# AntoineBlanot/LC2IS

Hardware: AMD Instinct MI355X
Metric: training-step images/sec (512x512, ADE20K-150) (higher is better)
Workload: dtype bf16; 1 GPU; BaseModelWithText ViT-B/16 + CLIP-text + decoder + fused head/CE train step, 512x512, 151 classes, text len 16, sgd; batch_per_gpu=32, global_batch=32, parallelism=dp1

## Files before the change

### include/lc2is_hip.h

```cpp
#ifndef LC2IS_HIP_H
#define LC2IS_HIP_H
#include <stddef.h>
#include <stdint.h>

#ifdef __cplusplus
extern "C" {
#endif

#define LC2IS_ACT_NONE 0
#define LC2IS_ACT_QUICK_GELU 1
#define LC2IS_ACT_RELU 2
#define LC2IS_ACT_DQUICK_GELU 3
#define LC2IS_ACT_DRELU 4
#define LC2IS_ACT_QUICK_GELU_GRAD 5
#define LC2IS_ACT_MUL_AUX 6
#define LC2IS_ACT_GELU_ERF 7
#define LC2IS_ACT_DGELU_ERF 8
#define LC2IS_ACT_ADD_AUX 9

#define LC2IS_INTERP_BICUBIC 0
#define LC2IS_INTERP_BILINEAR 1

typedef void* lc2is_stream_t;

// ... 108 lines not shown
  int C;
  int accumulate;
} lc2is_ln_partials;
int lc2is_layernorm_bwd_partials(int M, int C);
int lc2is_ln_partials_reduce(const lc2is_ln_partials* items, int n, lc2is_stream_t stream);

int lc2is_attention_fwd(const void* Q, int ldq, const void* K, int ldk, const void* V, int ldv, void* O,
                        int ldo, float* lse2, const float* kbias, int B, int H, int Sq, int Sk, int D,
                        float scale, int causal, lc2is_stream_t stream);

int lc2is_attention_bwd(const void* Q, int ldq, const void* K, int ldk, const void* V, int ldv,
                        const void* O, int ldo, const void* dO, int lddo, void* dQ, int lddq, void* dK,
                        int lddk, void* dV, int lddv, const float* lse2, float* delta, const float* kbias,
                        int B, int H, int Sq, int Sk, int D, float scale, int causal, lc2is_stream_t stream);

int lc2is_attention_fwd_dropout(const void* Q, int ldq, const void* K, int ldk, const void* V, int ldv, void* O,
                                int ldo, float* lse2, const float* kbias, int B, int H, int Sq, int Sk, int D,
                                float scale, int causal, float p_drop, unsigned long long seed, lc2is_stream_t stream);
int lc2is_attention_bwd_dropout(const void* Q, int ldq, const void* K, int ldk, const void* V, int ldv,
                                const void* O, int ldo, const void* dO, int lddo, void* dQ, int lddq, void* dK,
                                int lddk, void* dV, int lddv, const float* lse2, float* delta, const float* kbias,
                                int B, int H, int Sq, int Sk, int D, float scale, int causal, float p_drop,
                                unsigned long long seed, lc2is_stream_t stream);

int lc2is_dropout_rows_f32(const float* x, int ldx, const float* resid, int ldr, float* y32, int ldy, void* y16,
                           int ldy16, int M, int C, int rows_per_sample, float p, unsigned long long seed,
                           lc2is_stream_t stream);
int lc2is_dropout_rows_bf16(const void* x, int ldx, void* y, int ldy, int M, int C, float p, unsigned long long seed,
                            lc2is_stream_t stream);
int lc2is_dropout_mask(unsigned char* out, long rows, int cols, float p, unsigned long long seed, lc2is_stream_t stream);


int lc2is_shadow_refresh(const lc2is_shadow_desc* descs, int ndesc, int total_tiles, lc2is_stream_t stream);
int lc2is_cast_f32_bf16(const float* src, int ld_src, void* dst_bf16, int ld_dst, int M, int C,
                        lc2is_stream_t stream);
int lc2is_transpose_bf16(const void* src, int ld_src, void* dst, int ld_dst, int R, int C,
                         lc2is_stream_t stream);
int lc2is_transpose_bf16_batched(const void* src, int ld_src, long stride_src, void* dst, int ld_dst, long stride_dst,
                                 int R, int C, int batch, lc2is_stream_t stream);

int lc2is_patchify(const float* pixels, void* out_bf16, int ld_out, int B, int H, int W, int patch,
                   lc2is_stream_t stream);
int lc2is_vit_embed_fwd(const float* patch, int ld_patch, const float* cls, const float* pos, float* x,
                        int ldx, int B, int P, int C, lc2is_stream_t stream);
int lc2is_vit_embed_bwd(const float* dx, int ldx, float* dpos, float* dcls, void* dpatch_bf16, int ld_dpatch,
                        int B, int P, int C, int accumulate, lc2is_stream_t stream);
// ... 340 lines not shown
```

### lc2is_amd/nn/decoder.py

```python
from __future__ import annotations

import copy

import torch
from torch import nn

from .. import ops
from .base import (DropSites, HipModule, WgradBatch, drop_branch_add, drop_branch_grad16, grad_buf, linear_bwd_params,
                   require_cuda, vec_grad)


class _SelfAttnParams(nn.Module):
    def __init__(self, c, bias):
        super().__init__()
        self.in_proj_weight = nn.Parameter(torch.empty(3 * c, c))
        self.in_proj_bias = nn.Parameter(torch.zeros(3 * c)) if bias else None
        self.out_proj = nn.Linear(c, c, bias=bias)
        nn.init.xavier_uniform_(self.in_proj_weight)


class _CrossAttnParams(nn.Module):
    def __init__(self, c, ckv):
        super().__init__()
        self.q_proj_weight = nn.Parameter(torch.empty(c, c))
        self.k_proj_weight = nn.Parameter(torch.empty(c, ckv))
        self.v_proj_weight = nn.Parameter(torch.empty(c, ckv))
        self.in_proj_bias = nn.Parameter(torch.zeros(3 * c))
        self.out_proj = nn.Linear(c, c, bias=True)
        for w in (self.q_proj_weight, self.k_proj_weight, self.v_proj_weight):
            nn.init.xavier_uniform_(w)
        nn.init.zeros_(self.out_proj.bias)

# ... 46 lines not shown
    sa, ca = layer.self_attn, layer.multihead_attn
    s = dict(w_in=torch.empty(3 * C, C, **bf), w_inT=torch.empty(C, 3 * C, **bf),
             w_so=torch.empty(C, C, **bf), w_soT=torch.empty(C, C, **bf),
             w_q=torch.empty(C, C, **bf), w_qT=torch.empty(C, C, **bf),
             w_kv=torch.empty(2 * C, Ckv, **bf), w_kvT=torch.empty(Ckv, 2 * C, **bf),
             w_co=torch.empty(C, C, **bf), w_coT=torch.empty(C, C, **bf),
             w1=torch.empty(F, C, **bf), w1T=torch.empty(C, F, **bf),
             w2=torch.empty(C, F, **bf), w2T=torch.empty(F, C, **bf))
    e = [(sa.in_proj_weight, s["w_in"], s["w_inT"]), (sa.out_proj.weight, s["w_so"], s["w_soT"]),
         (ca.q_proj_weight, s["w_q"], s["w_qT"]),
         (ca.k_proj_weight, s["w_kv"][:C], s["w_kvT"][:, :C]), (ca.v_proj_weight, s["w_kv"][C:], s["w_kvT"][:, C:]),
         (ca.out_proj.weight, s["w_co"], s["w_coT"]),
         (layer.linear1.weight, s["w1"], s["w1T"]), (layer.linear2.weight, s["w2"], s["w2T"])]
    return s, e


def _layer_fwd(x, mem16, layer: DecoderLayer, s, B, Sq, Sk, kbias, save, ds: DropSites | None = None):
    C, H = layer.d_model, layer.nhead
    D = C // H
    scale = D ** -0.5
    sa, ca = layer.self_attn, layer.multihead_attn
    bq, bkv = ca.in_proj_bias[:C], ca.in_proj_bias[C:]
    nf = layer.norm_first
    sv = {}

    def ln(i, t, want_f32):
        n = getattr(layer, f"norm{i}")
        yb, yf, m, r = ops.layernorm_fwd(t, n.weight, n.bias, layer.eps, save_stats=save, out_bf16=True,
                                         out_f32=True if want_f32 else None)
        sv[f"ln{i}"] = (t, m, r)
        return yb, yf

    if nf:
        h1, _ = ln(1, x, False)
    else:
        h1 = ops.cast_bf16(x)
    qkv, _, _ = ops.gemm_nt(h1, s["w_in"], sa.in_proj_bias)
    pd = ds.p if ds is not None else 0.0
    o1, lse1 = ops.attention_fwd(qkv[:, :C], qkv[:, C:2 * C], qkv[:, 2 * C:], B, H, Sq, Sq, D, scale, save_lse=save,
                                 dropout_p=pd, seed=ds.seed("sa_p") if ds else 0)
    if ds is None:
        _, x1, _ = ops.gemm_nt(o1, s["w_so"], sa.out_proj.bias, resid=x, out_bf16=None, out_f32=True)
    else:
        _, br, _ = ops.gemm_nt(o1, s["w_so"], sa.out_proj.bias, out_bf16=None, out_f32=True)
        x1 = drop_branch_add(ds, "d1", br, x)
    if not nf:
        h2, x1 = ln(1, x1, True)
    if nf:
        h2, _ = ln(2, x1, False)
    q, _, _ = ops.gemm_nt(h2, s["w_q"], bq)
    kv, _, _ = ops.gemm_nt(mem16, s["w_kv"], bkv)
    o2, lse2 = ops.attention_fwd(q, kv[:, :C], kv[:, C:], B, H, Sq, Sk, D, scale, kbias=kbias, save_lse=save,
                                 dropout_p=pd, seed=ds.seed("ca_p") if ds else 0)
    if ds is None:
        _, x2, _ = ops.gemm_nt(o2, s["w_co"], ca.out_proj.bias, resid=x1, out_bf16=None, out_f32=True)
    else:
        _, br, _ = ops.gemm_nt(o2, s["w_co"], ca.out_proj.bias, out_bf16=None, out_f32=True)
        x2 = drop_branch_add(ds, "d2", br, x1)
    if not nf:
        h3, x2 = ln(2, x2, True)
    if nf:
        h3, _ = ln(3, x2, False)
    a, _, _ = ops.gemm_nt(h3, s["w1"], layer.linear1.bias, act=ops.ACT_RELU)
    if ds is None:
        _, x3, _ = ops.gemm_nt(a, s["w2"], layer.linear2.bias, resid=x2, out_bf16=None, out_f32=True)
    else:
        ops.dropout_rows_bf16(a, ds.p, ds.seed("ff"))
        _, br, _ = ops.gemm_nt(a, s["w2"], layer.linear2.bias, out_bf16=None, out_f32=True)
        x3 = drop_branch_add(ds, "d3", br, x2)
    if not nf:
        _, x3 = ln(3, x3, True)
    if save:
        sv.update(h1=h1, qkv=qkv, o1=o1, lse1=lse1, h2=h2, q=q, kv=kv, o2=o2, lse2=lse2, h3=h3, a=a, ds=ds)
    return x3, (sv if save else None)


def _layer_bwd(g32, g16, dmem32, mem16, layer, s, sv, B, Sq, Sk, kbias):
    with WgradBatch():
        return _layer_bwd_impl(g32, g16, dmem32, mem16, layer, s, sv, B, Sq, Sk, kbias)


def _layer_bwd_impl(g32, g16, dmem32, mem16, layer: DecoderLayer, s, sv, B, Sq, Sk, kbias):
    C, H = layer.d_model, layer.nhead
    D = C // H
    scale = D ** -0.5
    sa, ca = layer.self_attn, layer.multihead_attn
    nf = layer.norm_first

    def ln_bwd(i, dy, dres):
        n = getattr(layer, f"norm{i}")
        t, m, r = sv[f"ln{i}"]
        dg, accg = vec_grad(n.weight)
        db, _ = vec_grad(n.bias)
        a32, a16, _, _ = ops.layernorm_bwd(dy, t, n.weight, m, r, dres=dres, dgamma=dg, dbeta=db, accumulate=accg,
                                           need_param_grads=dg is not None)
        return a32, a16

    ds = sv.get("ds")
    pd = ds.p if ds is not None else 0.0
    if not nf:
        g32, g16 = ln_bwd(3, g32, None)
    gb16 = drop_branch_grad16(ds, "d3", g32, g16)
    linear_bwd_params(gb16, sv["a"], layer.linear2.weight, layer.linear2.bias)
    dz, _, _ = ops.gemm_nt(gb16, s["w2T"], None, act=ops.ACT_DRELU, aux_in=sv["a"])
    if ds is not None:
        ops.dropout_rows_bf16(dz, ds.p, ds.seeds["ff"])
    linear_bwd_params(dz, sv["h3"], layer.linear1.weight, layer.linear1.bias)
    if nf:
        dh3, _, _ = ops.gemm_nt(dz, s["w1T"], None)
        g32, g16 = ln_bwd(3, dh3, g32)
    else:
        _, g32, _ = ops.gemm_nt(dz, s["w1T"], None, resid=g32, out_bf16=None, out_f32=True)
        g32, g16 = ln_bwd(2, g32, None)
    gb16 = drop_branch_grad16(ds, "d2", g32, g16)
    linear_bwd_params(gb16, sv["o2"], ca.out_proj.weight, ca.out_proj.bias)
    do2, _, _ = ops.gemm_nt(gb16, s["w_coT"], None)
    q, kv = sv["q"], sv["kv"]
    dq = torch.empty_like(q)
    dkv = torch.empty_like(kv)
    ops.attention_bwd(q, kv[:, :C], kv[:, C:], sv["o2"], do2, sv["lse2"], B, H, Sq, Sk, D, scale, kbias=kbias, dq=dq,
                      dk=dkv[:, :C], dv=dkv[:, C:], dropout_p=pd, seed=ds.seeds["ca_p"] if ds else 0)
    gb, accb = vec_grad(ca.in_proj_bias)
    if ca.q_proj_weight.requires_grad:
        gw, acc = grad_buf(ca.q_proj_weight)
        ops.gemm_tn(dq, sv["h2"], gw, accumulate=acc)
        gw, acc = grad_buf(ca.k_proj_weight)
        ops.gemm_tn(dkv[:, :C], mem16, gw, accumulate=acc)
        gw, acc = grad_buf(ca.v_proj_weight)
        ops.gemm_tn(dkv[:, C:], mem16, gw, accumulate=acc)
    if gb is not None:
        ops.colsum(dq, gb[:C], accumulate=accb)
        ops.colsum(dkv, gb[C:], accumulate=accb)
    ops.gemm_nt(dkv, s["w_kvT"], None, resid=dmem32, out_bf16=None, out_f32=dmem32)
    if nf:
        dh2, _, _ = ops.gemm_nt(dq, s["w_qT"], None)
        g32, g16 = ln_bwd(2, dh2, g32)
    else:
        _, g32, _ = ops.gemm_nt(dq, s["w_qT"], None, resid=g32, out_bf16=None, out_f32=True)
        g32, g16 = ln_bwd(1, g32, None)
    gb16 = drop_branch_grad16(ds, "d1", g32, g16)
    linear_bwd_params(gb16, sv["o1"], sa.out_proj.weight, sa.out_proj.bias)
    do1, _, _ = ops.gemm_nt(gb16, s["w_soT"], None)
    qkv = sv["qkv"]
    dqkv = torch.empty_like(qkv)
    ops.attention_bwd(qkv[:, :C], qkv[:, C:2 * C], qkv[:, 2 * C:], sv["o1"], do1, sv["lse1"], B, H, Sq, Sq, D, scale,
                      dq=dqkv[:, :C], dk=dqkv[:, C:2 * C], dv=dqkv[:, 2 * C:], dropout_p=pd,
                      seed=ds.seeds["sa_p"] if ds else 0)
    linear_bwd_params(dqkv, sv["h1"], sa.in_proj_weight, sa.in_proj_bias)
    if nf:
        dh1, _, _ = ops.gemm_nt(dqkv, s["w_inT"], None)
        g32, g16 = ln_bwd(1, dh1, g32)
    else:
        _, g32, _ = ops.gemm_nt(dqkv, s["w_inT"], None, resid=g32, out_bf16=None, out_f32=True)
        g16 = ops.cast_bf16(g32)
# ... 101 lines not shown
```

### lc2is_amd/ops.py

```python
from __future__ import annotations

import ctypes as C
import math
import os

import torch

from . import _lib

ACT_NONE, ACT_QUICK_GELU, ACT_RELU, ACT_DQUICK_GELU, ACT_DRELU, ACT_QUICK_GELU_GRAD, ACT_MUL_AUX = 0, 1, 2, 3, 4, 5, 6
ACT_GELU_ERF, ACT_DGELU_ERF, ACT_ADD_AUX = 7, 8, 9

_P, _I, _F, _Z, _L, _U64 = C.c_void_p, C.c_int, C.c_float, C.c_size_t, C.c_long, C.c_ulonglong
_ARGTYPES = {
    "lc2is_gemm_nt_bf16": [_P, _I, _P, _I, _P, _P, _I, _P, _I, _P, _I, _P, _I, _P, _I, _I, _I, _I, _I, _I, _P],
    "lc2is_gemm_nt_plan": [_P, _I, _P, _I, _P, _P, _I, _P, _I, _P, _I, _P, _I, _P, _I, _I, _I, _I, _I, _I, _P, _I],
    "lc2is_gemm_nt_ln_xchg_bytes": [_I, _I],
    "lc2is_gemm_nt_ln_bf16": [_P, _I, _P, _I, _P, _P, _I, _P, _I, _P, _P, _F, _P, _I, _P, _P, _P, _Z, _I, _I, _I, _P],
    "lc2is_gemm_nt_bf16_batched": [_P, _I, _L, _P, _I, _L, _P, _I, _L, _P, _I, _L, _I, _I, _I, _I, _P],
    "lc2is_transpose_bf16_batched": [_P, _I, _L, _P, _I, _L, _I, _I, _I, _P],
    "lc2is_gemm_tn_workspace_bytes": [_I, _I, _I],
    "lc2is_gemm_tn_bf16": [_P, _I, _P, _I, _P, _I, _P, _I, _I, _I, _I, _P, _Z, _P],
    "lc2is_gemm_tn_plan": [_I, _I, _I, _P],
    "lc2is_gemm_tn_grouped_plan": [_P, _I, _P, _P, _I],
    "lc2is_colsum_workspace_bytes": [_I, _I],
    "lc2is_colsum_bf16": [_P, _I, _P, _I, _I, _I, _P, _Z, _P],
    "lc2is_layernorm_fwd": [_P, _I, _I, _P, _P, _P, _I, _P, _I, _P, _P, _I, _I, _F, _P],
    "lc2is_layernorm_bwd_partials": [_I, _I],
    "lc2is_ln_partials_reduce": [_P, _I, _P],
    "lc2is_layernorm_bwd_workspace_bytes": [_I, _I],
    "lc2is_layernorm_bwd": [_P, _I, _P, _I, _P, _I, _I, _P, _P, _P, _P, _I, _I, _P, _I, _P, _I, _P, _P, _I, _I, _I,
                            _P, _Z, _P],
    "lc2is_attention_fwd": [_P, _I, _P, _I, _P, _I, _P, _I, _P, _P, _I, _I, _I, _I, _I, _F, _I, _P],
    "lc2is_attention_bwd": [_P, _I, _P, _I, _P, _I, _P, _I, _P, _I, _P, _I, _P, _I, _P, _I, _P, _P, _P,
                            _I, _I, _I, _I, _I, _F, _I, _P],
    "lc2is_attention_fwd_dropout": [_P, _I, _P, _I, _P, _I, _P, _I, _P, _P, _I, _I, _I, _I, _I, _F, _I, _F, _U64, _P],
    "lc2is_attention_bwd_dropout": [_P, _I, _P, _I, _P, _I, _P, _I, _P, _I, _P, _I, _P, _I, _P, _I, _P, _P, _P,
                                    _I, _I, _I, _I, _I, _F, _I, _F, _U64, _P],
    "lc2is_dropout_rows_f32": [_P, _I, _P, _I, _P, _I, _P, _I, _I, _I, _I, _F, _U64, _P],
    "lc2is_dropout_rows_bf16": [_P, _I, _P, _I, _I, _I, _F, _U64, _P],
    "lc2is_dropout_mask": [_P, _L, _I, _F, _U64, _P],
    "lc2is_shadow_refresh": [_P, _I, _I, _P],
    "lc2is_set_cu_budget": [_I],
    "lc2is_get_cu_budget": [],
    "lc2is_cast_f32_bf16": [_P, _I, _P, _I, _I, _I, _P],
    "lc2is_transpose_bf16": [_P, _I, _P, _I, _I, _I, _P],
    "lc2is_patchify": [_P, _P, _I, _I, _I, _I, _I, _P],
    "lc2is_vit_embed_fwd": [_P, _I, _P, _P, _P, _I, _I, _I, _I, _P],
    "lc2is_vit_embed_bwd": [_P, _I, _P, _P, _P, _I, _I, _I, _I, _I, _P],
    "lc2is_text_embed_fwd": [_P, _P, _P, _P, _I, _I, _I, _I, _I, _P],
    "lc2is_text_embed_bwd": [_P, _P, _I, _P, _P, _I, _I, _I, _I, _I, _P],
    "lc2is_rows_copy_bf16": [_P, _I, _I, _P, _P, _I, _I, _I, _I, _I, _P],
    "lc2is_rows_copy_f32": [_P, _I, _I, _P, _P, _I, _I, _I, _I, _I, _P],
    "lc2is_sgd_step": [_P, _P, _P, _Z, _F, _F, _F, _F, _P],
    "lc2is_adamw_step": [_P, _P, _P, _P, _Z, _F, _F, _F, _F, _F, _I, _F, _P],
    "lc2is_grad_sumsq_blocks": [_Z],
    "lc2is_grad_sumsq_workspace_bytes": [_Z],
    "lc2is_grad_sumsq": [_P, _Z, _P, _Z, _P],
    "lc2is_optim_ctrl_update": [_P, _P, _P, _I, _P, _I, _F, _F, _I, _F, _F, _P],
    "lc2is_accum_add": [_P, _P, _P],
    "lc2is_optim_ctrl_update_accum": [_P, _P, _I, _P, _P, _I, _P, _I, _F, _F, _I, _F, _F, _P],
# ... 521 lines not shown
    while items:
        chunk, rest, seen = [], [], set()
        for it in items:
            outs = {t.data_ptr() for t in (it[3], it[4]) if t is not None}
            if len(chunk) < LN_PARTIALS_MAX and not (outs & seen) and not rest:
                chunk.append(it); seen |= outs
            else:
                rest.append(it)
        arr = (LnPartials * len(chunk))()
        for i, (ws, nparts, Cc, dg, db, acc) in enumerate(chunk):
            _chk(dg, torch.float32, "dgamma", 1); _chk(db, torch.float32, "dbeta", 1)
            arr[i] = LnPartials(_ptr(ws), _ptr(dg), _ptr(db), nparts, Cc, int(acc))
        rc = _fn("lc2is_ln_partials_reduce")(arr, len(chunk), _stream())
        _lib.check(rc, f"ln_partials_reduce n={len(chunk)}")
        items = rest


def ln_defer_end(prev):
    global _ln_defer
    ln_defer_flush()
    _ln_defer = prev


def attention_fwd(q: torch.Tensor, k: torch.Tensor, v: torch.Tensor, B: int, H: int, Sq: int, Sk: int, D: int,
                  scale: float, *, causal: bool = False, kbias: torch.Tensor | None = None,
                  save_lse: bool = True, out: torch.Tensor | None = None, dropout_p: float = 0.0, seed: int = 0):
    who, bf = "attention_fwd", torch.bfloat16
    dev, qs, ks = q.device, (B * Sq, H * D), (B * Sk, H * D)
    if _dims(who, q, "q", 2, bf) != qs:
        raise RuntimeError(f"lc2is_amd.attention_fwd: q must have shape {qs}, got {tuple(q.shape)}")
    _chk_op(who, k, "k", bf, ks, dev); _chk_op(who, v, "v", bf, ks, dev)
    _chk_op(who, kbias, "kbias", torch.float32, (B, Sk), dev, 4)
    o = out
    if o is None:
        o = torch.empty(qs, dtype=bf, device=dev)
    else:
        _chk_op(who, o, "out", bf, qs, dev); _chk_ld8(who, o, "out")
    lse = torch.empty((B, H, Sq), dtype=torch.float32, device=q.device) if save_lse else None
    if dropout_p > 0.0:
        rc = _fn("lc2is_attention_fwd_dropout")(_ptr(q), _ld(q), _ptr(k), _ld(k), _ptr(v), _ld(v), _ptr(o), _ld(o),
                                                _ptr(lse), _ptr(kbias), B, H, Sq, Sk, D, float(scale), int(causal),
                                                float(dropout_p), int(seed), _stream())
    else:
        rc = _fn("lc2is_attention_fwd")(_ptr(q), _ld(q), _ptr(k), _ld(k), _ptr(v), _ld(v), _ptr(o), _ld(o),
                                        _ptr(lse), _ptr(kbias), B, H, Sq, Sk, D, float(scale), int(causal),
                                        _stream())
    _lib.check(rc, f"attention_fwd B={B} H={H} Sq={Sq} Sk={Sk} D={D}")
    return o, lse


def attention_bwd(q, k, v, o, do, lse2, B: int, H: int, Sq: int, Sk: int, D: int, scale: float, *,
                  causal: bool = False, kbias: torch.Tensor | None = None, dq=None, dk=None, dv=None,
                  dropout_p: float = 0.0, seed: int = 0):
    who, bf = "attention_bwd", torch.bfloat16
    dev, qs, ks = q.device, (B * Sq, H * D), (B * Sk, H * D)
    if _dims(who, q, "q", 2, bf) != qs:
        raise RuntimeError(f"lc2is_amd.attention_bwd: q must have shape {qs}, got {tuple(q.shape)}")
    for t, n, s in ((k, "k", ks), (v, "v", ks), (o, "o", qs), (do, "do", qs)):
        if t is None:
            raise RuntimeError(f"lc2is_amd.attention_bwd: {n} is required")
        _chk_op(who, t, n, bf, s, dev)
    _chk_op(who, dq, "dq", bf, qs, dev); _chk_op(who, dk, "dk", bf, ks, dev); _chk_op(who, dv, "dv", bf, ks, dev)
    if dq is None:
        dq = torch.empty(qs, dtype=bf, device=dev)
    else:
        _chk_ld8(who, dq, "dq")
    dk = dk if dk is not None else torch.empty(ks, dtype=bf, device=dev)
    dv = dv if dv is not None else torch.empty(ks, dtype=bf, device=dev)
    if lse2 is None:
        raise RuntimeError("lc2is_amd.attention_bwd: lse2 is required")
    _chk_op(who, lse2, "lse2", torch.float32, (B, H, Sq), dev, 4); _chk_op(who, kbias, "kbias", torch.float32, (B, Sk), dev, 4)
    delta = torch.empty((B, H, Sq), dtype=torch.float32, device=dev)
    args = (_ptr(q), _ld(q), _ptr(k), _ld(k), _ptr(v), _ld(v), _ptr(o), _ld(o), _ptr(do), _ld(do), _ptr(dq), _ld(dq),
            _ptr(dk), _ld(dk), _ptr(dv), _ld(dv), _ptr(lse2), _ptr(delta), _ptr(kbias), B, H, Sq, Sk, D, float(scale),
            int(causal))
    if dropout_p > 0.0:
        rc = _fn("lc2is_attention_bwd_dropout")(*args, float(dropout_p), int(seed), _stream())
    else:
        rc = _fn("lc2is_attention_bwd")(*args, _stream())
    _lib.check(rc, f"attention_bwd B={B} H={H} Sq={Sq} Sk={Sk} D={D}")
    return dq, dk, dv


def dropout_rows_f32(x: torch.Tensor, p: float, seed: int, *, resid: torch.Tensor | None = None,
                     out_f32: torch.Tensor | bool | None = True, out_bf16: torch.Tensor | bool | None = None,
                     rows_per_sample: int = 0):
    who, dev = "dropout_rows_f32", x.device
    M, Cc = _dims(who, x, "x", 2, torch.float32)
    _chk_op(who, resid, "resid", torch.float32, (M, Cc), dev)
    yf = _out(out_f32, (M, Cc), torch.float32, dev)
    yb = _out(out_bf16, (M, Cc), torch.bfloat16, dev)
    if out_f32 is not True:
        _chk_op(who, yf, "out_f32", torch.float32, (M, Cc), dev)
    if out_bf16 is not True:
# ... 1630 lines not shown
```

Baseline: 1100 images/s.

## Add few-keys attention kernels and fuse decoder out-proj with layernorm

Adds specialised forward and backward attention kernels for short key sequences (Sk up to 64, D 64 or 96). Each block stages all of K and V for a head in LDS, computes the softmax in one pass with no online rescaling, and in backward accumulates dK/dV across query tiles in registers before a block reduction. This targets the decoder cross-attention over text tokens, where the generic flash kernel spends effort on key tiling. The decoder also fuses the out-projection GEMM with the residual add and the next layernorm, and moves the q-projection weight gradient into the batched wgrad group. Both new paths are behind env flags that default on.

```diff
diff --git a/include/lc2is_hip.h b/include/lc2is_hip.h
--- a/include/lc2is_hip.h
+++ b/include/lc2is_hip.h
@@ -154,6 +154,14 @@
                                 int lddk, void* dV, int lddv, const float* lse2, float* delta, const float* kbias,
                                 int B, int H, int Sq, int Sk, int D, float scale, int causal, float p_drop,
                                 unsigned long long seed, lc2is_stream_t stream);
+
+int lc2is_attention_fewkeys_fwd(const void* Q, int ldq, const void* K, int ldk, const void* V, int ldv, void* O,
+                                int ldo, float* lse2, const float* kbias, int B, int H, int Sq, int Sk, int D,
+                                float scale, int causal, lc2is_stream_t stream);
+int lc2is_attention_fewkeys_bwd(const void* Q, int ldq, const void* K, int ldk, const void* V, int ldv,
+                                const void* O, int ldo, const void* dO, int lddo, void* dQ, int lddq, void* dK,
+                                int lddk, void* dV, int lddv, const float* lse2, const float* kbias, int B, int H,
+                                int Sq, int Sk, int D, float scale, int causal, lc2is_stream_t stream);
 
 int lc2is_dropout_rows_f32(const float* x, int ldx, const float* resid, int ldr, float* y32, int ldy, void* y16,
                            int ldy16, int M, int C, int rows_per_sample, float p, unsigned long long seed,
diff --git a/lc2is_amd/csrc/attention_fewkeys.hip b/lc2is_amd/csrc/attention_fewkeys.hip
--- /dev/null
+++ b/lc2is_amd/csrc/attention_fewkeys.hip
@@ -0,0 +1,482 @@
+#include "attn_common.h"
+#include "lc2is_hip.h"
+
+namespace {
+
+constexpr float FK_LOG2E = 1.44269504088896341f;
+constexpr int FK_QB = 256;
+
+template <int D, int NKG> struct FkCfg {
+  static constexpr int PITCH = 2 * D + 16;
+  static constexpr int KR = 32 * NKG;
+  static constexpr int PP = 2 * KR + 16;
+  static constexpr int NKS = D / 16, NDT = D / 32, CPR = D / 8;
+  static constexpr int KV_BYTES = 2 * KR * PITCH + KR * 4;
+  static constexpr int FWD_LDS = KV_BYTES + 4 * 32 * PITCH;
+  static constexpr int BWD_WAVE = 64 * PITCH + 64 * PP;
+  static constexpr int RP = D + 4;
+  static constexpr int BWD_LDS = KV_BYTES + 4 * BWD_WAVE;
+  static_assert(2 * KR * RP * 4 <= BWD_LDS, "the dK / dV sum reuses the images");
+};
+
+__device__ __forceinline__ bf16x8_t fk_pack8(const f32x16_t& v, int r0) {
+  bf16x8_t o;
+#pragma unroll
+  for (int j = 0; j < 8; ++j) o[j] = (__bf16)v[r0 + j];
+  return o;
+}
+
+__device__ __forceinline__ float fk_dot8(const i32x4_t a, const i32x4_t b) {
+  float s = 0.f;
+#pragma unroll
+  for (int i = 0; i < 4; ++i) {
+    const unsigned x = (unsigned)a[i], y = (unsigned)b[i];
+    s += __builtin_bit_cast(float, x << 16) * __builtin_bit_cast(float, y << 16);
+    s += __builtin_bit_cast(float, x & 0xffff0000u) * __builtin_bit_cast(float, y & 0xffff0000u);
+  }
+  return s;
+}
+
+template <int D, int NKG>
+__device__ __forceinline__ void fk_stage_kv(char* smem, const bf16_t* K, int ldk, const bf16_t* V, int ldv, const float* kbias,
+                                            int B, int Sk, int b, int head, int tid) {
+  using C = FkCfg<D, NKG>;
+  const __amdgpu_buffer_rsrc_t rsK = make_rsrc(K, (unsigned)B * Sk * ldk * 2u);
+  const __amdgpu_buffer_rsrc_t rsV = make_rsrc(V, (unsigned)B * Sk * ldv * 2u);
+  for (int i = tid; i < C::KR * C::CPR; i += 256) {
+    const int r = i / C::CPR, ch = i - r * C::CPR;
+    const int ko = r < Sk ? ((b * Sk + r) * ldk + head * D + ch * 8) * 2 : -1;
+    const int vo = r < Sk ? ((b * Sk + r) * ldv + head * D + ch * 8) * 2 : -1;
+    *(i32x4_t*)(smem + r * C::PITCH + ch * 16) = __builtin_amdgcn_raw_buffer_load_b128(rsK, ko, 0, 0);
+    *(i32x4_t*)(smem + (C::KR + r) * C::PITCH + ch * 16) = __builtin_amdgcn_raw_buffer_load_b128(rsV, vo, 0, 0);
+  }
+  if (tid < C::KR) {
+    float* bias_l = (float*)(smem + 2 * C::KR * C::PITCH);
+    bias_l[tid] = tid < Sk ? (kbias ? kbias[(size_t)b * Sk + tid] * FK_LOG2E : 0.f) : -__builtin_inff();
+  }
+}
+
+template <int D, int PITCH>
+__device__ __forceinline__ void fk_store_rows(const char* img, bf16_t* dst, unsigned bytes, int tok0, int q0, int Sq, int ld,
+                                              int col0, int lane) {
+  constexpr int CPR = D / 8, RPI = 64 / CPR;
+  const __amdgpu_buffer_rsrc_t rs = make_rsrc(dst, bytes);
+  const int r_in = lane / CPR, ch = lane % CPR;
+  if (lane < RPI * CPR) {
+#pragma unroll
+    for (int it = 0; it < (32 + RPI - 1) / RPI; ++it) {
+      const int row = it * RPI + r_in;
+      if (row < 32) {
+        const i32x4_t v = *(const i32x4_t*)(img + row * PITCH + ch * 16);
+        const int off = (q0 + row < Sq) ? ((tok0 + q0 + row) * ld + col0 + ch * 8) * 2 : -1;
+        __builtin_amdgcn_raw_buffer_store_b128(v, rs, off, 0, 0);
+      }
+    }
+  }
+}
+
+struct FkFwdArgs {
+  const bf16_t* Q; int ldq;
+  const bf16_t* K; int ldk;
+  const bf16_t* V; int ldv;
+  bf16_t* O; int ldo;
+  float* lse2;
+  const float* kbias;
+  int B, H, Sq, Sk;
+  float scale_log2;
+};
+
+template <int D, int NKG>
+__global__ __launch_bounds__(256) void attn_fewkeys_fwd_kernel(FkFwdArgs p) {
+  using C = FkCfg<D, NKG>;
+  constexpr int PITCH = C::PITCH, KR = C::KR, NKS = C::NKS, NDT = C::NDT;
+  extern __shared__ __attribute__((aligned(16))) char smem[];
+  const int tid = threadIdx.x, lane = tid & 63;
+  const int wid = __builtin_amdgcn_readfirstlane(tid >> 6);
+  const int hh = lane >> 5, l31 = lane & 31;
+  const int q4 = (lane >> 2) & 3, p4 = lane & 3, cg = (lane >> 4) & 1;
+  const int nqb = (p.Sq + FK_QB - 1) / FK_QB;
+  const int bx = blockIdx.x % nqb, head = (blockIdx.x / nqb) % p.H, b = blockIdx.x / (nqb * p.H);
+  const float NEG_INF = -__builtin_inff();
+
+  fk_stage_kv<D, NKG>(smem, p.K, p.ldk, p.V, p.ldv, p.kbias, p.B, p.Sk, b, head, tid);
+  __syncthreads();
+
+  const unsigned smem_a = (unsigned)(size_t)LDS_PTR(smem);
+  const unsigned k_row = smem_a + l31 * PITCH + hh * 16;
+  const unsigned v_tr = smem_a + (KR + 4 * hh + q4) * PITCH + (16 * cg + 4 * p4) * 2;
+  char* obuf = smem + C::KV_BYTES + wid * (32 * PITCH);
+  float bias2[NKG][16];
+  {
+    const float* bias_l = (const float*)(smem + 2 * KR * PITCH);
+#pragma unroll
+    for (int g = 0; g < NKG; ++g)
+#pragma unroll
+      for (int c = 0; c < 4; ++c) {
+        const f32x4_t t = *(const f32x4_t*)(bias_l + 32 * g + 8 * c + 4 * hh);
+#pragma unroll
+        for (int j = 0; j < 4; ++j) bias2[g][4 * c + j] = t[j];
+      }
+  }
+
+  const __amdgpu_buffer_rsrc_t rsQ = make_rsrc(p.Q, (unsigned)p.B * p.Sq * p.ldq * 2u);
+  const int qend = (bx + 1) * FK_QB < p.Sq ? (bx + 1) * FK_QB : p.Sq;
+  auto load_q = [&](int q0, bf16x8_t (&qf)[NKS]) __attribute__((always_inline)) {
+    const int qr = q0 + l31;
+    const int off = (q0 < qend && qr < p.Sq) ? ((b * p.Sq + qr) * p.ldq + head * D + 8 * hh) * 2 : -1;
+#pragma unroll
+    for (int s = 0; s < NKS; ++s)
+      qf[s] = __builtin_bit_cast(bf16x8_t, __builtin_amdgcn_raw_buffer_load_b128(rsQ, off < 0 ? -1 : off + s * 32, 0, 0));
+  };
+
+  bf16x8_t qf[NKS], qn[NKS];
+  load_q(bx * FK_QB + wid * 32, qf);
+  for (int q0 = bx * FK_QB + wid * 32; q0 < qend; q0 += 128) {
+    load_q(q0 + 128, qn);
+    const int qrow = q0 + l31;
+    f32x16_t st[NKG];
+#pragma unroll
+    for (int g = 0; g < NKG; ++g) {
+#pragma unroll
+      for (int r = 0; r < 16; ++r) st[g][r] = 0.f;
+#pragma unroll
+      for (int s = 0; s < NKS; ++s)
+        st[g] = __builtin_amdgcn_mfma_f32_32x32x16_bf16(lds_read_b128(k_row + (unsigned)(32 * g * PITCH + 32 * s)), qf[s], st[g], 0, 0, 0);
+    }
+    float mx = NEG_INF;
+#pragma unroll
+    for (int g = 0; g < NKG; ++g)
+#pragma unroll
+      for (int r = 0; r < 16; ++r) {
+        st[g][r] = __builtin_fmaf(st[g][r], p.scale_log2, bias2[g][r]);
+        mx = fmaxf(mx, st[g][r]);
+      }
+    mx = fmaxf(mx, __shfl_xor(mx, 32, 64));
+    const float mref = mx == NEG_INF ? 0.f : mx;
+    float lsum = 0.f;
+#pragma unroll
+    for (int g = 0; g < NKG; ++g)
+#pragma unroll
+      for (int r = 0; r < 16; ++r) {
+        st[g][r] = __builtin_amdgcn_exp2f(st[g][r] - mref);
+        lsum += st[g][r];
+      }
+    const float l_tot = lsum + __shfl_xor(lsum, 32, 64);
+    f32x16_t ot[NDT];
+#pragma unroll
+    for (int d = 0; d < NDT; ++d)
+#pragma unroll
+      for (int r = 0; r < 16; ++r) ot[d][r] = 0.f;
+#pragma unroll
+    for (int g = 0; g < NKG; ++g)
+#pragma unroll
+      for (int s2 = 0; s2 < 2; ++s2) {
+        const bf16x8_t pf = fk_pack8(st[g], 8 * s2);
+#pragma unroll
+        for (int d = 0; d < NDT; ++d) {
+          const unsigned a = v_tr + (unsigned)((32 * g + 16 * s2) * PITCH + 64 * d);
+          ot[d] = __builtin_amdgcn_mfma_f32_32x32x16_bf16(tr_frag2a(a, a + 8 * PITCH), pf, ot[d], 0, 0, 0);
+        }
+      }
+    const float inv = l_tot > 0.f ? 1.f / l_tot : 0.f;
+    if (p.lse2 && hh == 0 && qrow < p.Sq)
+      p.lse2[((size_t)b * p.H + head) * p.Sq + qrow] = l_tot > 0.f ? mref + __builtin_amdgcn_logf(l_tot) : NEG_INF;
+#pragma unroll
+    for (int d = 0; d < NDT; ++d)
+#pragma unroll
+      for (int c = 0; c < 4; ++c) {
+        const int col = 32 * d + 8 * c + 4 * hh;
+        *(uint2*)(obuf + l31 * PITCH + col * 2) = make_uint2(pack_bf16x2(ot[d][4 * c] * inv, ot[d][4 * c + 1] * inv),
+                                                             pack_bf16x2(ot[d][4 * c + 2] * inv, ot[d][4 * c + 3] * inv));
+      }
+    fk_store_rows<D, PITCH>(obuf, p.O, (unsigned)p.B * p.Sq * p.ldo * 2u, b * p.Sq, q0, p.Sq, p.ldo, head * D, lane);
+#pragma unroll
+    for (int s = 0; s < NKS; ++s) qf[s] = qn[s];
+  }
+}
+
+struct FkBwdArgs {
+  const bf16_t* Q; int ldq;
+  const bf16_t* K; int ldk;
+  const bf16_t* V; int ldv;
+  const bf16_t* O; int ldo;
+  const bf16_t* dO; int lddo;
+  bf16_t* dQ; int lddq;
+  bf16_t* dK; int lddk;
+  bf16_t* dV; int lddv;
+  const float* lse2;
+  const float* kbias;
+  int B, H, Sq, Sk;
+  float scale, scale_log2;
+};
+
+template <int D, int NKG>
+__global__ __launch_bounds__(256) void attn_fewkeys_bwd_kernel(FkBwdArgs p) {
+  using C = FkCfg<D, NKG>;
+  constexpr int PITCH = C::PITCH, KR = C::KR, PP = C::PP, NKS = C::NKS, NDT = C::NDT, RP = C::RP;
+  extern __shared__ __attribute__((aligned(16))) char smem[];
+  const int tid = threadIdx.x, lane = tid & 63;
+  const int wid = __builtin_amdgcn_readfirstlane(tid >> 6);
+  const int hh = lane >> 5, l31 = lane & 31;
+  const int q4 = (lane >> 2) & 3, p4 = lane & 3, cg = (lane >> 4) & 1;
+  const int head = blockIdx.x % p.H, b = blockIdx.x / p.H;
+  const float INF = __builtin_inff();
+
+  fk_stage_kv<D, NKG>(smem, p.K, p.ldk, p.V, p.ldv, p.kbias, p.B, p.Sk, b, head, tid);
+  __syncthreads();
+
+  const unsigned smem_a = (unsigned)(size_t)LDS_PTR(smem);
+  const unsigned k_row = smem_a + l31 * PITCH + hh * 16;
+  const unsigned tr_d = (4 * hh + q4) * PITCH + (16 * cg + 4 * p4) * 2;
+  const unsigned tr_p = (4 * hh + q4) * PP + (16 * cg + 4 * p4) * 2;
+  char* wave = smem + C::KV_BYTES + wid * C::BWD_WAVE;
+  char* qimg = wave;
+  char* doimg = wave + 32 * PITCH;
+  char* pimg = wave + 64 * PITCH;
+  char* dsimg = pimg + 32 * PP;
+  const unsigned wave_a = smem_a + C::KV_BYTES + wid * C::BWD_WAVE;
+  const unsigned kt_tr = smem_a + tr_d, qt_tr = wave_a + tr_d, dot_tr = wave_a + 32 * PITCH + tr_d;
+  const unsigned pt_tr = wave_a + 64 * PITCH + tr_p, dst_tr = pt_tr + 32 * PP;
+  const float* bias_l = (const float*)(smem + 2 * KR * PITCH);
+
+  const __amdgpu_buffer_rsrc_t rsQ = make_rsrc(p.Q, (unsigned)p.B * p.Sq * p.ldq * 2u);
+  const __amdgpu_buffer_rsrc_t rsO = make_rsrc(p.O, (unsigned)p.B * p.Sq * p.ldo * 2u);
+  const __amdgpu_buffer_rsrc_t rsdO = make_rsrc(p.dO, (unsigned)p.B * p.Sq * p.lddo * 2u);
+  auto load_rows = [&](int q0, i32x4_t (&qv)[NKS], i32x4_t (&gv)[NKS], i32x4_t (&ov)[NKS]) __attribute__((always_inline)) {
+    const int qr = q0 + l31;
+    const bool ok = qr < p.Sq;
+    const int tok = b * p.Sq + qr;
+    const int qo = (tok * p.ldq + head * D + 8 * hh) * 2;
+    const int go = (tok * p.lddo + head * D + 8 * hh) * 2;
+    const int oo = (tok * p.ldo + head * D + 8 * hh) * 2;
+#pragma unroll
+    for (int s = 0; s < NKS; ++s) {
+      qv[s] = __builtin_amdgcn_raw_buffer_load_b128(rsQ, ok ? qo + s * 32 : -1, 0, 0);
+      gv[s] = __builtin_amdgcn_raw_buffer_load_b128(rsdO, ok ? go + s * 32 : -1, 0, 0);
+      ov[s] = __builtin_amdgcn_raw_buffer_load_b128(rsO, ok ? oo + s * 32 : -1, 0, 0);
+    }
+  };
+
+  f32x16_t dkt[NDT][NKG], dvt[NDT][NKG];
+#pragma unroll
+  for (int d = 0; d < NDT; ++d)
+#pragma unroll
+    for (int g = 0; g < NKG; ++g)
+#pragma unroll
+      for (int r = 0; r < 16; ++r) dkt[d][g][r] = dvt[d][g][r] = 0.f;
+
+  i32x4_t qv[NKS], gv[NKS], ov[NKS], qn[NKS], gn[NKS], on[NKS];
+  load_rows(wid * 32, qv, gv, ov);
+  for (int q0 = wid * 32; q0 < p.Sq; q0 += 128) {
+    const int qrow = q0 + l31;
+    float dpart = 0.f;
+#pragma unroll
+    for (int s = 0; s < NKS; ++s) dpart += fk_dot8(ov[s], gv[s]);
+    const float delta = dpart + __shfl_xor(dpart, 32, 64);
+    float lse = INF;
+    if (qrow < p.Sq) {
+      const float l = p.lse2[((size_t)b * p.H + head) * p.Sq + qrow];
+      lse = (l == -INF) ? INF : l;
+    }
+#pragma unroll
+    for (int s = 0; s < NKS; ++s) {
+      *(i32x4_t*)(qimg + l31 * PITCH + (2 * s + hh) * 16) = qv[s];
+      *(i32x4_t*)(doimg + l31 * PITCH + (2 * s + hh) * 16) = gv[s];
+    }
+    f32x16_t st[NKG], dpt[NKG];
+#pragma unroll
+    for (int g = 0; g < NKG; ++g) {
+#pragma unroll
+      for (int r = 0; r < 16; ++r) st[g][r] = dpt[g][r] = 0.f;
+#pragma unroll
+      for (int s = 0; s < NKS; ++s) {
+        const unsigned a = k_row + (unsigned)(32 * g * PITCH + 32 * s);
+        st[g] = __builtin_amdgcn_mfma_f32_32x32x16_bf16(lds_read_b128(a), __builtin_bit_cast(bf16x8_t, qv[s]), st[g], 0, 0, 0);
+        dpt[g] = __builtin_amdgcn_mfma_f32_32x32x16_bf16(lds_read_b128(a + KR * PITCH), __builtin_bit_cast(bf16x8_t, gv[s]), dpt[g], 0, 0, 0);
+      }
+    }
+    load_rows(q0 + 128, qn, gn, on);
+#pragma unroll
+    for (int g = 0; g < NKG; ++g)
+#pragma unroll
+      for (int c = 0; c < 4; ++c) {
+        const f32x4_t bs = *(const f32x4_t*)(bias_l + 32 * g + 8 * c + 4 * hh);
+#pragma unroll
+        for (int j = 0; j < 4; ++j) {
+          const int r = 4 * c + j;
+          const float pr = __builtin_amdgcn_exp2f(__builtin_fmaf(st[g][r], p.scale_log2, bs[j]) - lse);
+          st[g][r] = pr;
+          dpt[g][r] = pr * (dpt[g][r] - delta);
+        }
+        const int po = l31 * PP + (32 * g + 8 * c + 4 * hh) * 2;
+        *(uint2*)(pimg + po) = make_uint2(pack_bf16x2(st[g][4 * c], st[g][4 * c + 1]), pack_bf16x2(st[g][4 * c + 2], st[g][4 * c + 3]));
+        *(uint2*)(dsimg + po) = make_uint2(pack_bf16x2(dpt[g][4 * c], dpt[g][4 * c + 1]), pack_bf16x2(dpt[g][4 * c + 2], dpt[g][4 * c + 3]));
+      }
+    f32x16_t dq[NDT];
+#pragma unroll
+    for (int d = 0; d < NDT; ++d)
+#pragma unroll
+      for (int r = 0; r < 16; ++r) dq[d][r] = 0.f;
+#pragma unroll
+    for (int g = 0; g < NKG; ++g)
+#pragma unroll
+      for (int s2 = 0; s2 < 2; ++s2) {
+        const bf16x8_t dsf = fk_pack8(dpt[g], 8 * s2);
+#pragma unroll
+        for (int d = 0; d < NDT; ++d) {
+          const unsigned a = kt_tr + (unsigned)((32 * g + 16 * s2) * PITCH + 64 * d);
+          dq[d] = __builtin_amdgcn_mfma_f32_32x32x16_bf16(tr_frag2a(a, a + 8 * PITCH), dsf, dq[d], 0, 0, 0);
+        }
+      }
+#pragma unroll
+    for (int s2 = 0; s2 < 2; ++s2) {
+      bf16x8_t pT[NKG], dsT[NKG];
+#pragma unroll
+      for (int g = 0; g < NKG; ++g) {
+        const unsigned o = (unsigned)(16 * s2 * PP + 64 * g);
+        pT[g] = tr_frag2a(pt_tr + o, pt_tr + o + 8 * PP);
+        dsT[g] = tr_frag2a(dst_tr + o, dst_tr + o + 8 * PP);
+      }
+#pragma unroll
+      for (int d = 0; d < NDT; ++d) {
+        const unsigned o = (unsigned)(16 * s2 * PITCH + 64 * d);
+        const bf16x8_t doT = tr_frag2a(dot_tr + o, dot_tr + o + 8 * PITCH);
+        const bf16x8_t qT = tr_frag2a(qt_tr + o, qt_tr + o + 8 * PITCH);
+#pragma unroll
+        for (int g = 0; g < NKG; ++g) {
+          dvt[d][g] = __builtin_amdgcn_mfma_f32_32x32x16_bf16(doT, pT[g], dvt[d][g], 0, 0, 0);
+          dkt[d][g] = __builtin_amdgcn_mfma_f32_32x32x16_bf16(qT, dsT[g], dkt[d][g], 0, 0, 0);
+        }
+      }
+    }
+#pragma unroll
+    for (int d = 0; d < NDT; ++d)
+#pragma unroll
+      for (int c = 0; c < 4; ++c) {
+        const int col = 32 * d + 8 * c + 4 * hh;
+        *(uint2*)(qimg + l31 * PITCH + col * 2) = make_uint2(pack_bf16x2(dq[d][4 * c] * p.scale, dq[d][4 * c + 1] * p.scale),
+                                                             pack_bf16x2(dq[d][4 * c + 2] * p.scale, dq[d][4 * c + 3] * p.scale));
+      }
+    fk_store_rows<D, PITCH>(qimg, p.dQ, (unsigned)p.B * p.Sq * p.lddq * 2u, b * p.Sq, q0, p.Sq, p.lddq, head * D, lane);
+#pragma unroll
+    for (int s = 0; s < NKS; ++s) {
+      qv[s] = qn[s];
+      gv[s] = gn[s];
+      ov[s] = on[s];
+    }
+  }
+
+  __syncthreads();
+  float* red = (float*)smem;
+#pragma unroll 1
+  for (int w = 0; w < 4; ++w) {
+    if (wid == w) {
+#pragma unroll
+      for (int d = 0; d < NDT; ++d)
+#pragma unroll
+        for (int g = 0; g < NKG; ++g)
+#pragma unroll
+          for (int c = 0; c < 4; ++c) {
+            const int at = (32 * g + l31) * RP + 32 * d + 8 * c + 4 * hh;
+            f32x4_t* pk = (f32x4_t*)(red + at);
+            f32x4_t* pv = (f32x4_t*)(red + KR * RP + at);
+            const f32x4_t k4 = {dkt[d][g][4 * c], dkt[d][g][4 * c + 1], dkt[d][g][4 * c + 2], dkt[d][g][4 * c + 3]};
+            const f32x4_t v4 = {dvt[d][g][4 * c], dvt[d][g][4 * c + 1], dvt[d][g][4 * c + 2], dvt[d][g][4 * c + 3]};
+            if (w == 0) {
+              *pk = k4;
+              *pv = v4;
+            } else {
+              *pk += k4;
+              *pv += v4;
+            }
+          }
+    }
+    __syncthreads();
+  }
+  constexpr int D4 = D / 4;
+  for (int i = tid; i < 2 * p.Sk * D4; i += 256) {
+    const int which = i / (p.Sk * D4), rem = i - which * (p.Sk * D4);
+    const int key = rem / D4, d4 = (rem - key * D4) * 4;
+    f32x4_t v = *(const f32x4_t*)(red + (which * KR + key) * RP + d4);
+    if (!which) v *= p.scale;
+    bf16_t* dst = which ? p.dV + ((size_t)b * p.Sk + key) * p.lddv : p.dK + ((size_t)b * p.Sk + key) * p.lddk;
+    *(uint2*)(dst + head * D + d4) = make_uint2(pack_bf16x2(v[0], v[1]), pack_bf16x2(v[2], v[3]));
+  }
+}
+
+template <int D, int NKG>
+int launch_fk_fwd(const FkFwdArgs& a, hipStream_t stream) {
+  using C = FkCfg<D, NKG>;
+  if (int rc = set_dyn_lds<attn_fewkeys_fwd_kernel<D, NKG>>(C::FWD_LDS)) return rc;
+  const int nqb = (a.Sq + FK_QB - 1) / FK_QB;
+  hipLaunchKernelGGL((attn_fewkeys_fwd_kernel<D, NKG>), dim3(nqb * a.H * a.B), dim3(256), C::FWD_LDS, stream, a);
+  return lc2is_check_launch();
+}
+
+template <int D, int NKG>
+int launch_fk_bwd(const FkBwdArgs& a, hipStream_t stream) {
+  using C = FkCfg<D, NKG>;
+  if (int rc = set_dyn_lds<attn_fewkeys_bwd_kernel<D, NKG>>(C::BWD_LDS)) return rc;
+  hipLaunchKernelGGL((attn_fewkeys_bwd_kernel<D, NKG>), dim3(a.H * a.B), dim3(256), C::BWD_LDS, stream, a);
+  return lc2is_check_launch();
+}
+
+}
+
+extern "C" int lc2is_attention_fewkeys_fwd(const void* Q, int ldq, const void* K, int ldk, const void* V, int ldv, void* O,
+                                           int ldo, float* lse2, const float* kbias, int B, int H, int Sq, int Sk, int D,
+                                           float scale, int causal, lc2is_stream_t stream_) {
+  hipStream_t stream = (hipStream_t)stream_;
+  if (!Q || !K || !V || !O) return LC2IS_ERR_NULL;
+  if (B <= 0 || H <= 0 || Sq <= 0 || Sk <= 0) return LC2IS_ERR_SHAPE;
+  if (ldq < H * D || ldk < H * D || ldv < H * D || ldo < H * D || ldq % 8 || ldk % 8 || ldv % 8 || ldo % 8)
+    return LC2IS_ERR_SHAPE;
+  if (LC2IS_MISALIGNED(Q, 16) || LC2IS_MISALIGNED(K, 16) || LC2IS_MISALIGNED(V, 16) || LC2IS_MISALIGNED(O, 16) ||
+      LC2IS_MISALIGNED(lse2, 4) || LC2IS_MISALIGNED(kbias, 4))
+    return LC2IS_ERR_SHAPE;
+  if (causal || Sk > 64) return LC2IS_ERR_UNSUPPORTED;
+  const double lim = 2147483648.0;
+  if ((double)B * Sq * ldq * 2.0 >= lim || (double)B * Sq * ldo * 2.0 >= lim || (double)B * Sk * ldk * 2.0 >= lim ||
+      (double)B * Sk * ldv * 2.0 >= lim)
+    return LC2IS_ERR_UNSUPPORTED;
+  FkFwdArgs a{(const bf16_t*)Q, ldq, (const bf16_t*)K, ldk, (const bf16_t*)V, ldv, (bf16_t*)O, ldo, lse2, kbias,
+              B, H, Sq, Sk, scale * FK_LOG2E};
+  const bool one = Sk <= 32;
+  switch (D) {
+    case 64: return one ? launch_fk_fwd<64, 1>(a, stream) : launch_fk_fwd<64, 2>(a, stream);
+    case 96: return one ? launch_fk_fwd<96, 1>(a, stream) : launch_fk_fwd<96, 2>(a, stream);
+    default: return LC2IS_ERR_UNSUPPORTED;
+  }
+}
+
+extern "C" int lc2is_attention_fewkeys_bwd(const void* Q, int ldq, const void* K, int ldk, const void* V, int ldv,
+                                           const void* O, int ldo, const void* dO, int lddo, void* dQ, int lddq, void* dK,
+                                           int lddk, void* dV, int lddv, const float* lse2, const float* kbias, int B, int H,
+                                           int Sq, int Sk, int D, float scale, int causal, lc2is_stream_t stream_) {
+  hipStream_t stream = (hipStream_t)stream_;
+  if (!Q || !K || !V || !O || !dO || !dQ || !dK || !dV || !lse2) return LC2IS_ERR_NULL;
+  if (B <= 0 || H <= 0 || Sq <= 0 || Sk <= 0) return LC2IS_ERR_SHAPE;
+  const int hd = H * D;
+  if (ldq < hd || ldk < hd || ldv < hd || ldo < hd || lddo < hd || lddq < hd || lddk < hd || lddv < hd)
+    return LC2IS_ERR_SHAPE;
+  if (ldq % 8 || ldk % 8 || ldv % 8 || ldo % 8 || lddo % 8 || lddq % 8 || lddk % 4 || lddv % 4)
+    return LC2IS_ERR_SHAPE;
+  if (LC2IS_MISALIGNED(Q, 16) || LC2IS_MISALIGNED(K, 16) || LC2IS_MISALIGNED(V, 16) || LC2IS_MISALIGNED(O, 16) ||
+      LC2IS_MISALIGNED(dO, 16) || LC2IS_MISALIGNED(dQ, 16) || LC2IS_MISALIGNED_BF16(dK, lddk) || LC2IS_MISALIGNED_BF16(dV, lddv) ||
+      LC2IS_MISALIGNED(lse2, 4) || LC2IS_MISALIGNED(kbias, 4))
+    return LC2IS_ERR_SHAPE;
+  if (causal || Sk > 64) return LC2IS_ERR_UNSUPPORTED;
+  const double lim = 2147483648.0;
+  if ((double)B * Sq * ldq * 2.0 >= lim || (double)B * Sq * lddo * 2.0 >= lim || (double)B * Sq * ldo * 2.0 >= lim ||
+      (double)B * Sq * lddq * 2.0 >= lim || (double)B * Sk * ldk * 2.0 >= lim || (double)B * Sk * ldv * 2.0 >= lim)
+    return LC2IS_ERR_UNSUPPORTED;
+  FkBwdArgs a{(const bf16_t*)Q, ldq, (const bf16_t*)K, ldk, (const bf16_t*)V, ldv, (const bf16_t*)O, ldo,
+              (const bf16_t*)dO, lddo, (bf16_t*)dQ, lddq, (bf16_t*)dK, lddk, (bf16_t*)dV, lddv, lse2, kbias,
+              B, H, Sq, Sk, scale, scale * FK_LOG2E};
+  const bool one = Sk <= 32;
+  switch (D) {
+    case 64: return one ? launch_fk_bwd<64, 1>(a, stream) : launch_fk_bwd<64, 2>(a, stream);
+    case 96: return one ? launch_fk_bwd<96, 1>(a, stream) : launch_fk_bwd<96, 2>(a, stream);
+    default: return LC2IS_ERR_UNSUPPORTED;
+  }
+}
diff --git a/lc2is_amd/nn/decoder.py b/lc2is_amd/nn/decoder.py
--- a/lc2is_amd/nn/decoder.py
+++ b/lc2is_amd/nn/decoder.py
@@ -8,6 +8,8 @@
 from .. import ops
 from .base import (DropSites, HipModule, WgradBatch, drop_branch_add, drop_branch_grad16, grad_buf, linear_bwd_params,
                    require_cuda, vec_grad)
+
+_DECODER_FAST = __import__('os').environ.get("LC2IS_DECODER_FAST", "1") != "0"
 
 
 class _SelfAttnParams(nn.Module):
@@ -100,7 +102,15 @@
     sa, ca = layer.self_attn, layer.multihead_attn
     bq, bkv = ca.in_proj_bias[:C], ca.in_proj_bias[C:]
     nf = layer.norm_first
+    fast = _DECODER_FAST and nf and ds is None
+    fuse = fast and ops.gemm_nt_ln_ok(x.shape[0], C, C)
     sv = {}
+
+    def join_ln(i, a16, w, bias, resid):
+        n = getattr(layer, f"norm{i}")
+        xs, h, m, r = ops.gemm_nt_ln(a16, w, bias, resid, n.weight, n.bias, layer.eps, save_stats=save)
+        sv[f"ln{i}"] = (xs, m, r)
+        return xs, h
 
     def ln(i, t, want_f32):
         n = getattr(layer, f"norm{i}")
@@ -117,27 +127,33 @@
     pd = ds.p if ds is not None else 0.0
     o1, lse1 = ops.attention_fwd(qkv[:, :C], qkv[:, C:2 * C], qkv[:, 2 * C:], B, H, Sq, Sq, D, scale, save_lse=save,
                                  dropout_p=pd, seed=ds.seed("sa_p") if ds else 0)
-    if ds is None:
+    h2 = None
+    if fuse:
+        x1, h2 = join_ln(2, o1, s["w_so"], sa.out_proj.bias, x)
+    elif ds is None:
         _, x1, _ = ops.gemm_nt(o1, s["w_so"], sa.out_proj.bias, resid=x, out_bf16=None, out_f32=True)
     else:
         _, br, _ = ops.gemm_nt(o1, s["w_so"], sa.out_proj.bias, out_bf16=None, out_f32=True)
         x1 = drop_branch_add(ds, "d1", br, x)
     if not nf:
         h2, x1 = ln(1, x1, True)
-    if nf:
+    if nf and h2 is None:
         h2, _ = ln(2, x1, False)
     q, _, _ = ops.gemm_nt(h2, s["w_q"], bq)
     kv, _, _ = ops.gemm_nt(mem16, s["w_kv"], bkv)
     o2, lse2 = ops.attention_fwd(q, kv[:, :C], kv[:, C:], B, H, Sq, Sk, D, scale, kbias=kbias, save_lse=save,
                                  dropout_p=pd, seed=ds.seed("ca_p") if ds else 0)
-    if ds is None:
+    h3 = None
+    if fuse:
+        x2, h3 = join_ln(3, o2, s["w_co"], ca.out_proj.bias, x1)
+    elif ds is None:
         _, x2, _ = ops.gemm_nt(o2, s["w_co"], ca.out_proj.bias, resid=x1, out_bf16=None, out_f32=True)
     else:
         _, br, _ = ops.gemm_nt(o2, s["w_co"], ca.out_proj.bias, out_bf16=None, out_f32=True)
         x2 = drop_branch_add(ds, "d2", br, x1)
     if not nf:
         h3, x2 = ln(2, x2, True)
-    if nf:
+    if nf and h3 is None:
         h3, _ = ln(3, x2, False)
     a, _, _ = ops.gemm_nt(h3, s["w1"], layer.linear1.bias, act=ops.ACT_RELU)
     if ds is None:
@@ -149,7 +165,7 @@
     if not nf:
         _, x3 = ln(3, x3, True)
     if save:
-        sv.update(h1=h1, qkv=qkv, o1=o1, lse1=lse1, h2=h2, q=q, kv=kv, o2=o2, lse2=lse2, h3=h3, a=a, ds=ds)
+        sv.update(h1=h1, qkv=qkv, o1=o1, lse1=lse1, h2=h2, q=q, kv=kv, o2=o2, lse2=lse2, h3=h3, a=a, ds=ds, fast=fast)
     return x3, (sv if save else None)
 
 
@@ -164,6 +180,9 @@
     scale = D ** -0.5
     sa, ca = layer.self_attn, layer.multihead_attn
     nf = layer.norm_first
+
+    ds = sv.get("ds")
+    fast = bool(sv.get("fast"))
 
     def ln_bwd(i, dy, dres):
         n = getattr(layer, f"norm{i}")
@@ -174,7 +193,6 @@
                                            need_param_grads=dg is not None)
         return a32, a16
 
-    ds = sv.get("ds")
     pd = ds.p if ds is not None else 0.0
     if not nf:
         g32, g16 = ln_bwd(3, g32, None)
@@ -199,15 +217,22 @@
     ops.attention_bwd(q, kv[:, :C], kv[:, C:], sv["o2"], do2, sv["lse2"], B, H, Sq, Sk, D, scale, kbias=kbias, dq=dq,
                       dk=dkv[:, :C], dv=dkv[:, C:], dropout_p=pd, seed=ds.seeds["ca_p"] if ds else 0)
     gb, accb = vec_grad(ca.in_proj_bias)
+    q_bias_done = False
     if ca.q_proj_weight.requires_grad:
         gw, acc = grad_buf(ca.q_proj_weight)
-        ops.gemm_tn(dq, sv["h2"], gw, accumulate=acc)
+        batch = WgradBatch._active
+        if fast and batch is not None and ops.gemm_tn_groupable(dq, sv["h2"]) and (gb is None or accb == acc):
+            batch.items.append((dq, sv["h2"], gw, None if gb is None else gb[:C], acc))
+            q_bias_done = True
+        else:
+            ops.gemm_tn(dq, sv["h2"], gw, accumulate=acc)
         gw, acc = grad_buf(ca.k_proj_weight)
         ops.gemm_tn(dkv[:, :C], mem16, gw, accumulate=acc)
         gw, acc = grad_buf(ca.v_proj_weight)
         ops.gemm_tn(dkv[:, C:], mem16, gw, accumulate=acc)
     if gb is not None:
-        ops.colsum(dq, gb[:C], accumulate=accb)
+        if not q_bias_done:
+            ops.colsum(dq, gb[:C], accumulate=accb)
         ops.colsum(dkv, gb[C:], accumulate=accb)
     ops.gemm_nt(dkv, s["w_kvT"], None, resid=dmem32, out_bf16=None, out_f32=dmem32)
     if nf:
diff --git a/lc2is_amd/ops.py b/lc2is_amd/ops.py
--- a/lc2is_amd/ops.py
+++ b/lc2is_amd/ops.py
@@ -37,6 +37,9 @@
     "lc2is_attention_fwd_dropout": [_P, _I, _P, _I, _P, _I, _P, _I, _P, _P, _I, _I, _I, _I, _I, _F, _I, _F, _U64, _P],
     "lc2is_attention_bwd_dropout": [_P, _I, _P, _I, _P, _I, _P, _I, _P, _I, _P, _I, _P, _I, _P, _I, _P, _P, _P,
                                     _I, _I, _I, _I, _I, _F, _I, _F, _U64, _P],
+    "lc2is_attention_fewkeys_fwd": [_P, _I, _P, _I, _P, _I, _P, _I, _P, _P, _I, _I, _I, _I, _I, _F, _I, _P],
+    "lc2is_attention_fewkeys_bwd": [_P, _I, _P, _I, _P, _I, _P, _I, _P, _I, _P, _I, _P, _I, _P, _I, _P, _P,
+                                    _I, _I, _I, _I, _I, _F, _I, _P],
     "lc2is_dropout_rows_f32": [_P, _I, _P, _I, _P, _I, _P, _I, _I, _I, _I, _F, _U64, _P],
     "lc2is_dropout_rows_bf16": [_P, _I, _P, _I, _I, _I, _F, _U64, _P],
     "lc2is_dropout_mask": [_P, _L, _I, _F, _U64, _P],
@@ -604,6 +607,16 @@
     _ln_defer = prev
 
 
+ATTN_GENERIC, ATTN_FEWKEYS = "generic", "fewkeys"
+_ATTN_FEWKEYS = os.environ.get("LC2IS_ATTN_FEWKEYS", "1") != "0"
+
+
+def attention_plan(Sq: int, Sk: int, D: int, causal: bool = False, dropout_p: float = 0.0) -> str:
+    if _ATTN_FEWKEYS and 1 <= Sk <= 64 and Sq >= 1 and not causal and not dropout_p > 0.0 and D in (64, 96):
+        return ATTN_FEWKEYS
+    return ATTN_GENERIC
+
+
 def attention_fwd(q: torch.Tensor, k: torch.Tensor, v: torch.Tensor, B: int, H: int, Sq: int, Sk: int, D: int,
                   scale: float, *, causal: bool = False, kbias: torch.Tensor | None = None,
                   save_lse: bool = True, out: torch.Tensor | None = None, dropout_p: float = 0.0, seed: int = 0):
@@ -619,7 +632,10 @@
     else:
         _chk_op(who, o, "out", bf, qs, dev); _chk_ld8(who, o, "out")
     lse = torch.empty((B, H, Sq), dtype=torch.float32, device=q.device) if save_lse else None
-    if dropout_p > 0.0:
+    if attention_plan(Sq, Sk, D, causal, dropout_p) == ATTN_FEWKEYS:
+        rc = _fn("lc2is_attention_fewkeys_fwd")(_ptr(q), _ld(q), _ptr(k), _ld(k), _ptr(v), _ld(v), _ptr(o), _ld(o),
+                                                _ptr(lse), _ptr(kbias), B, H, Sq, Sk, D, float(scale), 0, _stream())
+    elif dropout_p > 0.0:
         rc = _fn("lc2is_attention_fwd_dropout")(_ptr(q), _ld(q), _ptr(k), _ld(k), _ptr(v), _ld(v), _ptr(o), _ld(o),
                                                 _ptr(lse), _ptr(kbias), B, H, Sq, Sk, D, float(scale), int(causal),
                                                 float(dropout_p), int(seed), _stream())
@@ -652,6 +668,12 @@
     if lse2 is None:
         raise RuntimeError("lc2is_amd.attention_bwd: lse2 is required")
     _chk_op(who, lse2, "lse2", torch.float32, (B, H, Sq), dev, 4); _chk_op(who, kbias, "kbias", torch.float32, (B, Sk), dev, 4)
+    if attention_plan(Sq, Sk, D, causal, dropout_p) == ATTN_FEWKEYS:
+        rc = _fn("lc2is_attention_fewkeys_bwd")(_ptr(q), _ld(q), _ptr(k), _ld(k), _ptr(v), _ld(v), _ptr(o), _ld(o), _ptr(do),
+                                                _ld(do), _ptr(dq), _ld(dq), _ptr(dk), _ld(dk), _ptr(dv), _ld(dv), _ptr(lse2),
+                                                _ptr(kbias), B, H, Sq, Sk, D, float(scale), 0, _stream())
+        _lib.check(rc, f"attention_bwd (few keys) B={B} H={H} Sq={Sq} Sk={Sk} D={D}")
+        return dq, dk, dv
     delta = torch.empty((B, H, Sq), dtype=torch.float32, device=dev)
     args = (_ptr(q), _ld(q), _ptr(k), _ld(k), _ptr(v), _ld(v), _ptr(o), _ld(o), _ptr(do), _ld(do), _ptr(dq), _ld(dq),
             _ptr(dk), _ld(dk), _ptr(dv), _ld(dv), _ptr(lse2), _ptr(delta), _ptr(kbias), B, H, Sq, Sk, D, float(scale),
```

After: 1106 images/s, median of 6. Within noise of the previous version (+0.5%).
